# DLR-RM/curvature

Measured on AMD Instinct MI355X. Metric: KFAC factor-build + invert + sample throughput, higher is better.
Workload: dtype f32

## Files before the change

### curvature_amd/csrc/invert.hip

```cpp
#include <type_traits>
#include "kernarg.h"
#include "mma64.h"
#include <hip/hip_ext.h>

#include <algorithm>
#include <chrono>
#include <cstdlib>
#include <mutex>
#include <vector>

namespace curv {

constexpr int INV_THREADS = MMA_THREADS;
constexpr int SQ_FLAGS = 32;
constexpr int SQ_FD = 0, SQ_FLC = 4, SQ_FLROW = 8, SQ_FT = 12;
constexpr int SQ_SPIN_LIMIT = 1 << 21;
#ifdef CURV_SQ_TRACE
__device__ long long g_sq_trace[256];
#define KT_BEGIN(slot) { if (threadIdx.x == 0 && k0 == 4 * (CURV_SQ_TRACE - 1)) atomicMax((unsigned long long*)&g_sq_trace[slot], (1ull << 62) - (unsigned long long)wall_clock64()); }
#define KT_END(slot) { if (threadIdx.x == 0 && k0 == 4 * (CURV_SQ_TRACE - 1)) atomicMax((unsigned long long*)&g_sq_trace[slot], (unsigned long long)wall_clock64()); }
#define SQT(slot) { if (threadIdx.x == 0 && f == 0 && stamp == CURV_SQ_TRACE) g_sq_trace[slot] = wall_clock64(); }
#define FIT(k) { if (threadIdx.x == 0 && trace_base >= 0) g_sq_trace[trace_base + (k)] = wall_clock64(); }
#else
#define SQT(slot)
// ... 786 lines not shown
__device__ __forceinline__ void sq_wait(int* flag, int stamp, int* lost) {
  if (threadIdx.x == 0) {
    int n = 0;
    while (__hip_atomic_load(flag, __ATOMIC_RELAXED, __HIP_MEMORY_SCOPE_AGENT) < stamp) {
      __builtin_amdgcn_s_sleep(2);
      if (++n > SQ_SPIN_LIMIT || *lost) { *lost = 1; break; }
    }
  }
  __syncthreads();
}

__global__ void __launch_bounds__(INV_THREADS)
chol_square_kernel(const InvDev* __restrict__ t, int nf, int k0, int kend, int* __restrict__ flags, int stamp) {
  __shared__ double Ds[NB * LDA], Is[NB * LDA], Bf[NB * LDA];
  __shared__ int bad, lost;
  int f, r;
  if (!locate(t, nf, blockIdx.x, [k0, kend](const InvDev& d) { return d.P > k0 ? (kend < d.P ? kend : d.P) - k0 : 0; }, f, r))
    return;
  const InvDev& d = t[f];
  const int np = d.np, tid = threadIdx.x;
  const int nbf = (kend < d.P ? kend : d.P) - k0;
  gdouble* W = (gdouble*)d.W;
  gdouble* X = (gdouble*)d.X;
  int* fl = flags + (long long)f * SQ_FLAGS;
  const int lane = tid & 63, wave = tid >> 6, wm = wave >> 1, wn = wave & 1;
  auto Wt = [&](int i, int j) { return W + (long long)(k0 + i) * NB * np + (k0 + j) * NB; };
  auto Xt = [&](int i, int j) { return X + (long long)(k0 + i) * NB * np + (k0 + j) * NB; };
  if (tid == 0) { bad = 0; lost = 0; }
  __syncthreads();
  f64x4 acc[2][2];
  if (r == 0) {
    SQT(0)
#ifdef CURV_SQ_TRACE
    if (tid == 0 && f == 0 && stamp == CURV_SQ_TRACE + 1) g_sq_trace[238] = wall_clock64();
#endif
    load_block(Wt(0, 0), np, Ds);
    if (nbf > 1) load_block(Wt(1, 0), np, Bf);
    __syncthreads();
    SQT(1)
    for (int q = 0; q < nbf; ++q) {
      if (q >= 1) {
        if (q >= 2) {
          sq_wait(fl + SQ_FT + q, stamp, &lost);
          SQT(8 * q + 0)
          load_block_coh(Wt(q, q - 1), np, Bf);
        }
        load_block_coh(Wt(q, q), np, Ds);
        __syncthreads();
        SQT(8 * q + 1)
        zero_acc(acc);
        mma_64_pre<true>(Bf, Is, wm, wn, lane, acc);
        SQT(8 * q + 2)
        store_acc_coh(Wt(q, q - 1), np, acc, wm, wn, lane, 1.0);
        __syncthreads();
        acc_to_lds(acc, wm, wn, lane, Bf);
        __syncthreads();
        zero_acc(acc);
        mma_64_pre<true>(Bf, Bf, wm, wn, lane, acc);
        lds_sub_acc(Ds, acc, wm, wn, lane);
        SQT(8 * q + 3)
        sq_signal(fl + SQ_FLC + q, stamp);
        SQT(8 * q + 4)
      }
#ifdef CURV_SQ_TRACE
      factor_invert_64(Ds, Is, &bad, (k0 + q) * NB, d.pivot_min, (f == 0 && stamp == CURV_SQ_TRACE) ? 112 + 4 * q : -1);
#else
      factor_invert_64(Ds, Is, &bad, (k0 + q) * NB, d.pivot_min);
#endif
      SQT(q == 0 ? 2 : 8 * q + 5)
      store_block_coh(Xt(q, q), np, Is);
      sq_signal(fl + SQ_FD + q, stamp);
      SQT(q == 0 ? 3 : 8 * q + 6)
    }
    if (tid == 0 && bad != 0) atomicCAS(d.info, 0, bad);
    if (tid == 0 && lost != 0) atomicCAS(d.info, 0, -1);
    return;
  }
  double* Af = Ds;
  SQT(64 * r + 0)
  double* Cf = Is;
  if (r >= 2) {
    f64x4 accA[2][2], accT0[2][2], accT1[2][2];
    zero_acc(accA); zero_acc(accT0); zero_acc(accT1);
    auto push = [&](int mp, int m) {
      load_block_coh(Wt(mp, m), np, Bf);
      __syncthreads();
      if (mp == 1) mma_64_pre<true>(Cf, Bf, wm, wn, lane, accT0);
      else mma_64_pre<true>(Cf, Bf, wm, wn, lane, accT1);
      __syncthreads();
    };
    for (int m = 0; m <= r - 2; ++m) {
      SQT(64 * r + 8 + 4 * m)
      load_block(Wt(r, m), np, Af);
      __syncthreads();
      if (m == 1) lds_sub_acc(Af, accT0, wm, wn, lane);
      sq_wait(fl + SQ_FD + m, stamp, &lost);
      SQT(64 * r + 9 + 4 * m)
      load_block_coh(Xt(m, m), np, Bf);
      __syncthreads();
      zero_acc(acc);
      mma_64_pre<true>(Af, Bf, wm, wn, lane, acc);
      SQT(64 * r + 10 + 4 * m)
      store_acc_coh(Wt(r, m), np, acc, wm, wn, lane, 1.0);
      acc_to_lds(acc, wm, wn, lane, Cf);
      if (m == r - 2) sq_signal(fl + SQ_FLROW + r, stamp);
      else __syncthreads();
      mma_64_pre<true>(Cf, Cf, wm, wn, lane, accA);
      __syncthreads();
      for (int mp = m + 1; mp <= r - 1; ++mp) {
        if (m == r - 2 && mp == r - 1) break;
        sq_wait(fl + (mp == m + 1 ? SQ_FLC : SQ_FLROW) + mp, stamp, &lost);
        push(mp, m);
      }
    }
    load_block(Wt(r, r), np, Bf);
    __syncthreads();
    lds_sub_acc(Bf, accA, wm, wn, lane);
    __syncthreads();
    store_block_coh(Wt(r, r), np, Bf);
    load_block(Wt(r, r - 1), np, Af);
    sq_wait(fl + SQ_FLC + r - 1, stamp, &lost);
    push(r - 1, r - 2);
    if (r == 2) lds_sub_acc(Af, accT0, wm, wn, lane);
    else lds_sub_acc(Af, accT1, wm, wn, lane);
    __syncthreads();
    store_block_coh(Wt(r, r - 1), np, Af);
    sq_signal(fl + SQ_FT + r, stamp);
    SQT(64 * r + 1)
  }
  {
    const int j = r - 1;
    for (int i = r; i < nbf; ++i) {
      f64x4 S[2][2];
      zero_acc(S);
      for (int m = j; m < i; ++m) {
        if (m == i - 1) sq_wait(fl + SQ_FLC + i, stamp, &lost);
        else sq_wait(fl + SQ_FLROW + i, stamp, &lost);
        if (m == j) sq_wait(fl + SQ_FD + j, stamp, &lost);
        load_block_coh(Wt(i, m), np, Af);
        load_block_coh(Xt(m, j), np, Bf);
        __syncthreads();
        mma_64_pre<false>(Af, Bf, wm, wn, lane, S);
        __syncthreads();
      }
      SQT(64 * r + 2 + 16 * (i - r))
      acc_to_lds(S, wm, wn, lane, Af);
      sq_wait(fl + SQ_FD + i, stamp, &lost);
      SQT(64 * r + 3 + 16 * (i - r))
      load_block_coh(Xt(i, i), np, Bf);
      __syncthreads();
      zero_acc(acc);
      mma_64_pre<false>(Bf, Af, wm, wn, lane, acc);
      store_acc_coh(Xt(i, j), np, acc, wm, wn, lane, -1.0);
      asm volatile("s_waitcnt vmcnt(0)" ::: "memory");
      __syncthreads();
      SQT(64 * r + 4 + 16 * (i - r))
    }
  }
  if (tid == 0 && lost != 0) atomicCAS(d.info, 0, -1);
}

__device__ __host__ __forceinline__ int panel_jobs(int P, int kind, int k0, int kend) {
  if (P <= k0) return 0;
  return (P > kend ? P - kend : 0) + (kind == 2 ? (kend < P ? kend : P) : kind == 1 ? k0 : 0);
}
template <int WV>
__device__ __forceinline__ void panel_product_body(const InvDev* __restrict__ t, int nf, int k0, int kend,
                                                   double* __restrict__ As, double* __restrict__ Bs) {
  int f, local;
  if (!locate(t, nf, blockIdx.x, [k0, kend](const InvDev& d) { return panel_jobs(d.P, s_kind(d), k0, kend); }, f, local))
    return;
  const InvDev& d = t[f];
  const int np = d.np, nb = (kend < d.P ? kend : d.P) - k0;
  gdouble* W = (gdouble*)d.W;
  gdouble* X = (gdouble*)d.X;
  TileJob o;
  o.np = np;
  o.same = false;
  o.ke0 = 0;
  const int n_below = d.P > kend ? d.P - kend : 0;
  const bool below = local < n_below;
  const int i = kend + local, j = local - n_below;
  o.bt = below;
  o.mode = below ? 1 : 3;
  gdouble* Zm = (gdouble*)d.Zm;
  const bool rhs = !below && Zm != nullptr;
  gdouble* S = rhs ? Zm : X;
  if (rhs) { o.mode = 1; o.ke0 = (j > k0 ? j - k0 : 0) * NB; }
  gfloat* C32 = below ? (gfloat*)d.C32 : nullptr;
  for (int c = nb - 1; c >= 0; --c) {
    if (rhs && k0 + c < j) break;
    const gdouble* xsq = X + (long long)(k0 + c) * NB * np + k0 * NB;
    o.a0 = below ? (const gbyte*)(W + (long long)i * NB * np + k0 * NB) : (const gbyte*)xsq;
    o.b0 = below ? (const gbyte*)xsq : (const gbyte*)(S + (long long)k0 * NB * np + j * NB);
    o.C = below ? W + (long long)i * NB * np + (k0 + c) * NB : S + (long long)(k0 + c) * NB * np + j * NB;
    o.C32 = C32 != nullptr ? C32 + (long long)i * NB * np + (k0 + c) * NB : nullptr;
    o.ke1 = (c + 1) * NB;
    tile_product_k32<WV>(o, As, Bs);
  }
}

constexpr int PQ_PITCH = 4 * NB + 1;
constexpr int PQ_OWN = 16 * PQ_PITCH > 4 * NB * 17 ? 16 * PQ_PITCH : 4 * NB * 17;
template <bool below>
__device__ __forceinline__ void panel_quarter_body(const InvDev& d, int k0, int nb, int i, int j, int q,
                                                   double* __restrict__ Own, double* __restrict__ Ts) {
  const int np = d.np;
  const int tid = threadIdx.x, lane = tid & 63, wave = tid >> 6, r16 = lane & 15, kq = lane >> 4;
  PQT(240)
  const gbyte* Wb = (const gbyte*)d.W;
  const gbyte* Xb = (const gbyte*)d.X;
  if (below) {
    const gbyte* g = Wb + (((long long)i * NB + 16 * q) * np + (long long)k0 * NB) * 8;
    for (int v = 0; v < nb; ++v) {
      double x[4];
#pragma unroll
      for (int u = 0; u < 4; ++u) x[u] = *(const gdouble*)(g + ((long long)((tid >> 6) + 4 * u) * np + (tid & 63) + 64 * v) * 8);
#pragma unroll
      for (int u = 0; u < 4; ++u) Own[((tid >> 6) + 4 * u) * PQ_PITCH + (tid & 63) + 64 * v] = x[u];
    }
  } else {
    const gbyte* g = Xb + ((long long)k0 * NB * np + (long long)j * NB + 16 * q) * 8;
    for (int v = 0; v < nb; ++v) {
      double x[4];
#pragma unroll
      for (int u = 0; u < 4; ++u) {
        x[u] = *(const gdouble*)(g + ((long long)((tid >> 4) + 16 * u + 64 * v) * np + (tid & 15)) * 8);
      }
#pragma unroll
      for (int u = 0; u < 4; ++u) Own[((tid >> 4) + 16 * u + 64 * v) * 17 + (tid & 15)] = x[u];
    }
  }
  double rt0[16], rt1[16], rt2[16];
  auto fetch = [&](int c, int kb, double (&rt)[16]) __attribute__((always_inline)) {
    const gbyte* g = Xb + (((long long)(k0 + c) * NB) * np + (long long)(k0 + kb) * NB) * 8;
#pragma unroll
    for (int u = 0; u < 16; ++u) rt[u] = *(const gdouble*)(g + ((long long)((tid >> 6) + 4 * u) * np + (tid & 63)) * 8);
  };
  auto next = [](int& c, int& kb) { if (++kb > c) { --c; kb = 0; } };
  int c = nb - 1, kb = 0;
  int cf = c, kf = kb;
  fetch(cf, kf, rt0); next(cf, kf);
  if (cf >= 0) { fetch(cf, kf, rt1); next(cf, kf); }
  if (cf >= 0) { fetch(cf, kf, rt2); next(cf, kf); }
  f64x4 acc[4] = {};
  PQT(241)
  [[maybe_unused]] int pq_n = 0;
  auto step = [&](double (&rt)[16]) __attribute__((always_inline)) {
    __syncthreads();
#pragma unroll
    for (int u = 0; u < 16; ++u) Ts[((tid >> 6) + 4 * u) * LDA + (tid & 63)] = rt[u];
    __syncthreads();
    if (cf >= 0) { fetch(cf, kf, rt); next(cf, kf); }
#pragma unroll
    for (int ks = 0; ks < NB / 4; ++ks) {
      const int k = 4 * ks + kq;
      const double a = below ? Own[r16 * PQ_PITCH + 64 * kb + k] : Ts[(16 * wave + r16) * LDA + k];
      const double b = below ? Ts[(16 * wave + r16) * LDA + k] : Own[(64 * kb + k) * 17 + r16];
      acc[ks & 3] = __builtin_amdgcn_mfma_f64_16x16x4f64(a, b, acc[ks & 3], 0, 0, 0);
    }
    if (kb == c) {
      const int wm = below ? q : wave, wn = below ? wave : q;
      const int c16 = lane & 15, rq = lane >> 4;
      gbyte* base = below ? (gbyte*)d.W + (((long long)i * NB) * np + (long long)(k0 + c) * NB) * 8
                          : (gbyte*)d.X + (((long long)(k0 + c) * NB) * np + (long long)j * NB) * 8;
      const unsigned voff = (unsigned)(((long long)(16 * wm + rq) * np + 16 * wn + c16) * 8);
      gbyte* base32 = (below && d.C32 != nullptr) ? (gbyte*)d.C32 + (((long long)i * NB) * np + (long long)(k0 + c) * NB) * 4 : nullptr;
      const unsigned voff32 = (unsigned)(((long long)(16 * wm + rq) * np + 16 * wn + c16) * 4);
#pragma unroll
      for (int qq = 0; qq < 4; ++qq) {
        const double v = (acc[0][qq] + acc[1][qq]) + (acc[2][qq] + acc[3][qq]);
        *(gdouble*)(base + (long long)(4 * qq) * np * 8 + voff) = below ? v : -v;
        if (below && base32 != nullptr) *(gfloat*)(base32 + (long long)(4 * qq) * np * 4 + voff32) = (float)v;
      }
#pragma unroll
      for (int u = 0; u < 4; ++u) acc[u] = f64x4{0.0, 0.0, 0.0, 0.0};
    }
    next(c, kb);
    PQT(242 + pq_n)
    ++pq_n;
  };
  while (c >= 0) {
    step(rt0);
    if (c < 0) break;
    step(rt1);
    if (c < 0) break;
    step(rt2);
  }
}
__global__ void __launch_bounds__(INV_THREADS)
panel_product_quarter_kernel(const InvDev* __restrict__ t, int nf, int k0, int kend) {
  __shared__ double Own[PQ_OWN], Ts[NB * LDA];
  const int job = (blockIdx.x >> 5) * 8 + (blockIdx.x & 7), q = (blockIdx.x >> 3) & 3;
  int f, local;
  KT_BEGIN(236)
  if (!locate(t, nf, job, [k0, kend](const InvDev& d) { return panel_jobs(d.P, s_kind(d), k0, kend); }, f, local)) return;
  const InvDev& d = t[f];
  const int nb = (kend < d.P ? kend : d.P) - k0;
  const int n_below = d.P > kend ? d.P - kend : 0;
  if (local < n_below) panel_quarter_body<true>(d, k0, nb, kend + local, 0, q, Own, Ts);
  else panel_quarter_body<false>(d, k0, nb, 0, local - n_below, q, Own, Ts);
  KT_END(237)
}
__global__ void __launch_bounds__(INV_THREADS, 3)
panel_product_kernel(const InvDev* __restrict__ t, int nf, int k0, int kend) {
  __shared__ double As[NB * OPA], Bs[NB * OPA > OKS * LDA ? NB * OPA : OKS * LDA];
  panel_product_body<2>(t, nf, k0, kend, As, Bs);
}
__global__ void __launch_bounds__(1024)
panel_product_wide_kernel(const InvDev* __restrict__ t, int nf, int k0, int kend) {
  __shared__ double As[NB * OPA], Bs[NB * OPA > OKS * LDA ? NB * OPA : OKS * LDA];
  panel_product_body<4>(t, nf, k0, kend, As, Bs);
}

constexpr int SKS = 32;
constexpr int SPA = SKS + 1;
constexpr int SPB = NB + 32;
struct Tile32 {
  const gbyte* a;
  const gbyte* b;
  gfloat* out;
  int np, ke0, ke1;
  bool a64, b64, accumulate, negate;
};
__device__ __forceinline__ void tile32(const Tile32& o, float* __restrict__ As, float* __restrict__ Bs) {
  const int np = o.np;
  const int tid = threadIdx.x, lane = tid & 63, wave = tid >> 6, wm = wave >> 1, wn = wave & 1;
  const int l32 = lane & 31, h = lane >> 5;
  const long long a_off = (long long)(tid >> 3) * np + 4 * (tid & 7), a_step = 32ll * np;
  const long long b_off = (long long)(tid >> 4) * np + 4 * (tid & 15), b_step = 16ll * np;
  typedef const __attribute__((address_space(1))) f32x4 gf4;
  typedef const __attribute__((address_space(1))) f64x4 gd4;
  f32x4 ra[2], rb[2];
  auto fetch = [&](int ke) __attribute__((always_inline)) {
    if (o.a64) {
#pragma unroll
      for (int u = 0; u < 2; ++u) {
        const f64x4 v = *(gd4*)(o.a + (a_off + u * a_step + ke) * 8);
        ra[u] = f32x4{(float)v[0], (float)v[1], (float)v[2], (float)v[3]};
      }
    } else {
#pragma unroll
      for (int u = 0; u < 2; ++u) ra[u] = *(gf4*)(o.a + (a_off + u * a_step + ke) * 4);
    }
    if (o.b64) {
#pragma unroll
      for (int u = 0; u < 2; ++u) {
        const f64x4 v = *(gd4*)(o.b + (b_off + u * b_step + (long long)ke * np) * 8);
        rb[u] = f32x4{(float)v[0], (float)v[1], (float)v[2], (float)v[3]};
      }
    } else {
#pragma unroll
      for (int u = 0; u < 2; ++u) rb[u] = *(gf4*)(o.b + (b_off + u * b_step + (long long)ke * np) * 4);
    }
  };
  f32x16 acc = {0};
  fetch(o.ke0);
  for (int ke = o.ke0; ke < o.ke1; ke += SKS) {
#pragma unroll
    for (int u = 0; u < 2; ++u)
#pragma unroll
      for (int e = 0; e < 4; ++e) {
        As[((tid >> 3) + 32 * u) * SPA + 4 * (tid & 7) + e] = ra[u][e];
        Bs[((tid >> 4) + 16 * u) * SPB + 4 * (tid & 15) + e] = rb[u][e];
      }
    __syncthreads();
    if (ke + SKS < o.ke1) fetch(ke + SKS);
#pragma unroll
    for (int kk = 0; kk < SKS; kk += 2) {
      const float av = As[(32 * wm + l32) * SPA + kk + h];
      const float bv = Bs[(kk + h) * SPB + 32 * wn + l32];
      acc = __builtin_amdgcn_mfma_f32_32x32x2f32(av, bv, acc, 0, 0, 0);
    }
    __syncthreads();
  }
  gbyte* base = (gbyte*)(o.out + (long long)(32 * wm + 4 * h) * np + 32 * wn + l32);
  if (!o.accumulate) {
#pragma unroll
    for (int reg = 0; reg < 16; ++reg)
      *(gfloat*)(base + (long long)((reg & 3) + 8 * (reg >> 2)) * np * 4) = o.negate ? -acc[reg] : acc[reg];
  } else {
    float old[16];
#pragma unroll
    for (int reg = 0; reg < 16; ++reg) old[reg] = *(const gfloat*)(base + (long long)((reg & 3) + 8 * (reg >> 2)) * np * 4);
#pragma unroll
    for (int reg = 0; reg < 16; ++reg) *(gfloat*)(base + (long long)((reg & 3) + 8 * (reg >> 2)) * np * 4) = old[reg] + acc[reg];
  }
}
__device__ __host__ __forceinline__ long long supd_tiles(int P, int kind, int kend) {
  if (kind != 0 || P <= kend) return 0;
  const long long nsb = (P - kend + SB - 1) / SB, ncb = (kend + SB - 1) / SB;
  return nsb * ncb * (SB * SB);
}
__global__ void __launch_bounds__(INV_THREADS, 3)
supd32_kernel(const InvDev* __restrict__ t, int nf, int k0, int kend, int n_items) {
  __shared__ float As[NB * SPA], Bs[SKS * SPB];
  int item;
  {
    const int bid = blockIdx.x, xcd = bid & 7, jj = bid >> 3;
    item = ((jj / (SB * SB)) * 8 + xcd) * (SB * SB) + (jj % (SB * SB));
  }
  if (item >= n_items) return;
  int f, local;
  if (!locate(t, nf, item, [kend](const InvDev& d) { return (int)supd_tiles(d.P, s_kind(d), kend); }, f, local)) return;
  const InvDev& d = t[f];
  const int np = d.np, r = d.P - kend;
  const int ncb = (kend + SB - 1) / SB;
  const int sb = local / (SB * SB), in = local - sb * (SB * SB);
  const int a = sb / ncb, cb = sb - a * ncb;
  const int ri = a * SB + in / SB, j = cb * SB + in % SB;
  if (ri >= r || j >= kend) return;
  const int i = kend + ri;
  const bool own = j >= k0;
  Tile32 o;
  o.np = np;
  o.a = (const gbyte*)((const gfloat*)d.C32 + (long long)i * NB * np);
  o.a64 = false;
  o.b = own ? (const gbyte*)((const gdouble*)d.X + j * NB) : (const gbyte*)((const gfloat*)d.X32 + j * NB);
  o.b64 = own;
  o.ke0 = (own ? j : k0) * NB;
  o.ke1 = kend * NB;
  o.out = (gfloat*)d.S32 + (long long)i * NB * np + j * NB;
  o.accumulate = !own;
  o.negate = false;
  tile32(o, As, Bs);
}
__device__ __host__ __forceinline__ long long xrow_tiles(int P, int kind, int k0, int kend) {
  if (kind != 0 || P <= k0) return 0;
  return (long long)((kend < P ? kend : P) - k0) * k0;
}
__global__ void __launch_bounds__(INV_THREADS, 3)
xrows32_kernel(const InvDev* __restrict__ t, int nf, int k0, int kend) {
  __shared__ float As[NB * SPA], Bs[SKS * SPB];
  int f, local;
  if (!locate(t, nf, blockIdx.x, [k0, kend](const InvDev& d) { return (int)xrow_tiles(d.P, s_kind(d), k0, kend); }, f, local)) return;
  const InvDev& d = t[f];
  const int np = d.np, nb = (kend < d.P ? kend : d.P) - k0;
  const int j = local / nb, c = nb - 1 - (local - j * nb);
  Tile32 o;
  o.np = np;
  o.a = (const gbyte*)((const gdouble*)d.X + (long long)(k0 + c) * NB * np);
  o.a64 = true;
  o.b = (const gbyte*)((const gfloat*)d.S32 + j * NB);
  o.b64 = false;
  o.ke0 = k0 * NB;
  o.ke1 = (k0 + c + 1) * NB;
  o.out = (gfloat*)d.X32 + (long long)(k0 + c) * NB * np + j * NB;
  o.accumulate = false;
  o.negate = true;
  tile32(o, As, Bs);
}

__global__ void __launch_bounds__(INV_THREADS)
inv_finalize_kernel(const InvDev* __restrict__ t, int nf, int sq) {
  __shared__ float tile[NB][NB + 1];
  int f, local;
  if (!locate(t, nf, blockIdx.x, [](const InvDev& d) { return d.P * d.P; }, f, local)) return;
  const InvDev& d = t[f];
  const int n = d.n, np = d.np, q = d.P;
  const int ti = local / q, tj = local - ti * q;
  const gdouble* X = (const gdouble*)d.X;
  const gfloat* X32 = (const gfloat*)d.X32;
  gfloat* L = (gfloat*)d.L;
  const int w = __builtin_amdgcn_readfirstlane(threadIdx.x >> 6), c = threadIdx.x & 63;
  if (!d.reverse) {
    gdouble* Xo = (gdouble*)d.Xout;
    const gdouble* S = d.Zm != nullptr ? (const gdouble*)d.Zm : X;
#pragma unroll 4
    for (int u = 0; u < 16; ++u) {
      const int i = ti * NB + w + 4 * u, j = tj * NB + c;
      if (i < n && j < n) {
        double v = (j <= i) ? S[(long long)i * np + j] : 0.0;
        if (d.r_minus && j <= i) v = ((const gdouble*)d.R)[(long long)i * n + j] - v;
        Xo[(long long)i * n + j] = v;
      }
    }
    return;
  }
  if (tj > ti) {
#pragma unroll 4
    for (int u = 0; u < 16; ++u) {
      const int i = ti * NB + w + 4 * u, j = tj * NB + c;
      if (i < n && j < n) L[(long long)i * n + j] = 0.0f;
    }
    return;
  }
  double xv[16];
  const int i_l = ti * NB + c;
#pragma unroll
  for (int u = 0; u < 16; ++u) {
    const int j = tj * NB + w + 4 * u;
    const int rs = n - 1 - j, cs = n - 1 - i_l;
    const bool live = i_l < n && j < n && j <= i_l;
    if (X32 == nullptr || rs / sq == cs / sq) xv[u] = live ? X[(long long)rs * np + cs] : 0.0;
    else xv[u] = live ? (double)X32[(long long)rs * np + cs] : 0.0;
  }
#pragma unroll
  for (int u = 0; u < 16; ++u) tile[w + 4 * u][c] = (float)xv[u];
  __syncthreads();
#pragma unroll
  for (int u = 0; u < 16; ++u) {
    const int i = ti * NB + w + 4 * u, j = tj * NB + c;
    if (i < n && j < n) L[(long long)i * n + j] = tile[c][w + 4 * u];
  }
}

constexpr int INV_UPLOAD_CHUNK = 28;

static size_t inv_table_bytes(int n) { return align_up((size_t)std::max(n, 1) * sizeof(InvDev), 256); }
static size_t inv_flags_bytes(int n) { return align_up((size_t)std::max(n, 1) * SQ_FLAGS * sizeof(int), 256); }

struct SideStream {
  hipStream_t stream = nullptr;
  hipEvent_t ev_main[2] = {nullptr, nullptr};
  hipEvent_t ev_side[2] = {nullptr, nullptr};
  hipEvent_t ev_tail = nullptr;
};
struct StreamSet {
  SideStream side[2];
  hipStream_t aux = nullptr;
  hipStream_t masked = nullptr;
  hipEvent_t ev_fork = nullptr, ev_join = nullptr, ev_join2 = nullptr;
  hipEvent_t ev_chain[2] = {nullptr, nullptr};
};
static std::mutex g_masked_mutex;
static std::vector<std::pair<int, hipStream_t>> g_masked_streams;
static void destroy_masked_streams() {
  std::lock_guard<std::mutex> lock(g_masked_mutex);
  for (auto& e : g_masked_streams) {
    if (hipSetDevice(e.first) == hipSuccess) {
      (void)hipStreamSynchronize(e.second);
      (void)hipStreamDestroy(e.second);
    }
  }
  g_masked_streams.clear();
}

static int stream_set(StreamSet** out) {
  static thread_local std::vector<std::pair<int, StreamSet>> cache;
  int dev = 0;
  CURV_HIP_CHECK(hipGetDevice(&dev));
  for (auto& e : cache) if (e.first == dev) { *out = &e.second; return CURV_OK; }
  StreamSet s;
  int prio_low = 0, prio_high = 0;
  CURV_HIP_CHECK(hipDeviceGetStreamPriorityRange(&prio_low, &prio_high));
  CURV_HIP_CHECK(hipEventCreateWithFlags(&s.ev_fork, hipEventDisableTiming));
  CURV_HIP_CHECK(hipEventCreateWithFlags(&s.ev_join, hipEventDisableTiming));
  CURV_HIP_CHECK(hipEventCreateWithFlags(&s.ev_join2, hipEventDisableTiming));
  for (int g = 0; g < 2; ++g) CURV_HIP_CHECK(hipEventCreateWithFlags(&s.ev_chain[g], hipEventDisableTiming));
  auto wide_stream = [&](hipStream_t* out) -> int {
    static const int free_cus = getenv("CURV_FREE_CUS") ? atoi(getenv("CURV_FREE_CUS")) : 32;
    hipDeviceProp_t prop;
    int dev_id = 0;
    CURV_HIP_CHECK(hipGetDevice(&dev_id));
    CURV_HIP_CHECK(hipGetDeviceProperties(&prop, dev_id));
    const int n_cu = prop.multiProcessorCount;
    if (free_cus > 0 && 2 * free_cus <= n_cu) {
      std::vector<uint32_t> mask((size_t)cdiv(n_cu, 32), 0u);
      for (int c = 0; c < n_cu - free_cus; ++c) mask[c >> 5] |= 1u << (c & 31);
      if (hipExtStreamCreateWithCUMask(out, (uint32_t)mask.size(), mask.data()) == hipSuccess) {
        std::lock_guard<std::mutex> lock(g_masked_mutex);
        if (g_masked_streams.empty()) atexit(destroy_masked_streams);
        g_masked_streams.emplace_back(dev_id, *out);
        return CURV_OK;
      }
      (void)hipGetLastError();
    }
    CURV_HIP_CHECK(hipStreamCreateWithPriority(out, hipStreamNonBlocking, prio_low));
    return CURV_OK;
  };
  CURV_HIP_CHECK(hipStreamCreateWithPriority(&s.aux, hipStreamNonBlocking, prio_high));
  CURV_HIP_CHECK(hipStreamCreateWithFlags(&s.masked, hipStreamNonBlocking));
  for (int g = 0; g < 2; ++g) {
    { const int rc = wide_stream(&s.side[g].stream); if (rc != CURV_OK) return rc; }
    for (int i = 0; i < 2; ++i) {
      CURV_HIP_CHECK(hipEventCreateWithFlags(&s.side[g].ev_main[i], hipEventDisableTiming));
      CURV_HIP_CHECK(hipEventCreateWithFlags(&s.side[g].ev_side[i], hipEventDisableTiming));
    }
    CURV_HIP_CHECK(hipEventCreateWithFlags(&s.side[g].ev_tail, hipEventDisableTiming));
  }
  cache.emplace_back(dev, s);
  *out = &cache.back().second;
  return CURV_OK;
}

int curv_internal_side_stream(hipStream_t* out) {
  StreamSet* ss = nullptr;
  const int rc = stream_set(&ss);
  if (rc != CURV_OK) return rc;
  *out = ss->masked;
  return CURV_OK;
}

}

using namespace curv;

#ifdef CURV_SQ_TRACE
extern "C" int curv_debug_sq_trace_reset() {
  long long zeros[256] = {0};
  return hipMemcpyToSymbol(HIP_SYMBOL(curv::g_sq_trace), zeros, sizeof(zeros)) == hipSuccess ? 0 : 1;
}
extern "C" int curv_debug_sq_trace(long long* out) {
  return hipMemcpyFromSymbol(out, HIP_SYMBOL(curv::g_sq_trace), 256 * sizeof(long long)) == hipSuccess ? 0 : 1;
}
#endif

extern "C" int curv_init_streams(void) {
  StreamSet* ss = nullptr;
  return stream_set(&ss);
}

extern "C" size_t curv_chol_inv_workspace_bytes(const curv_inv_desc* descs, int n_factors) {
  size_t total = 2 * inv_table_bytes(n_factors) + 2 * inv_flags_bytes(n_factors);
  for (int i = 0; i < n_factors; ++i) {
    if (descs[i].n <= 0) return 0;
    const size_t np = (size_t)cdiv(descs[i].n, NB) * NB;
    total += 2 * np * np * sizeof(double) + 3 * np * np * sizeof(float);
  }
  return total;
}

static int sweep_nbo(bool latency_bound) { return latency_bound ? 4 : 6; }
struct GroupSweep {
  hipStream_t stream;
  SideStream* side;
  const std::vector<InvDev>* tabp;
  InvDev* table;
  int* flags;
  bool latency_bound;
  int n_factors = 0, Pmax = 0, NBO = 4, k0 = 0, panel = 0;
  long long fin_tiles = 0, quarter_prod = 0;
  bool use_square = false, far_pending = false, inv_pending = false, capturing = false;

  GroupSweep(hipStream_t st, SideStream* sd, const std::vector<InvDev>& tab, InvDev* tb, int* fl, bool lb)
      : stream(st), side(sd), tabp(&tab), table(tb), flags(fl), latency_bound(lb) {}
  bool done() const { return k0 >= Pmax; }
  int panels() const { return cdiv(Pmax, NBO); }

  int begin() {
    const std::vector<InvDev>& tab = *tabp;
    n_factors = (int)tab.size();
    hipStreamCaptureStatus cap = hipStreamCaptureStatusNone;
    CURV_HIP_CHECK(hipStreamIsCapturing(stream, &cap));
    capturing = cap != hipStreamCaptureStatusNone;
    long long prep_tiles = 0;
    for (const InvDev& d : tab) {
      Pmax = std::max(Pmax, d.P);
      prep_tiles += (long long)d.P * (d.P + 1) / 2;
      fin_tiles += (long long)d.P * d.P;
    }
    const int rcu = upload_table<INV_UPLOAD_CHUNK>(stream, table, tab.data(), n_factors);
    if (rcu != CURV_OK) return rcu;
    hipLaunchKernelGGL(inv_prepare_kernel, dim3((unsigned)prep_tiles), dim3(INV_THREADS), 0, stream, table, n_factors, flags);
    CURV_LAUNCH_CHECK();
    NBO = sweep_nbo(latency_bound);
    return CURV_OK;
  }

  int panel_step() {
    const std::vector<InvDev>& tab = *tabp;
    constexpr long long WIDE_NEAR = 512, WIDE_PROD = 256;
    constexpr long long QUARTER_PROD = 512;
    quarter_prod = latency_bound ? QUARTER_PROD : 0;
    use_square = latency_bound;
    const int kend = k0 + NBO, row0 = kend + NBO;
    long long prod_tiles = 0;
    if (use_square) {
      long long sq_wgs = 0;
      for (const InvDev& d : tab)
        if (d.P > k0) sq_wgs += std::min(kend, d.P) - k0;
      hipLaunchKernelGGL(chol_square_kernel, dim3((unsigned)sq_wgs), dim3(INV_THREADS), 0, stream, table, n_factors, k0, kend,
                         flags, panel + 1);
      CURV_LAUNCH_CHECK();
    }
    for (int k = k0; !use_square && k < std::min(kend, Pmax); ++k) {
      long long diag_tiles = 0, panel_tiles = 0, upd_tiles = 0;
      for (const InvDev& d : tab) {
        if (d.P > k) { ++diag_tiles; panel_tiles += std::min(kend, d.P) - k0 - 1; }
        upd_tiles += inner_tiles(d.P, k, k0, kend);
      }
      if (k == k0) {
        hipLaunchKernelGGL(chol_diag_kernel, dim3((unsigned)diag_tiles), dim3(INV_THREADS), 0, stream, table, n_factors, k);
        CURV_LAUNCH_CHECK();
      }
      if (panel_tiles > 0) {
        hipLaunchKernelGGL(chol_panel_kernel, dim3((unsigned)panel_tiles), dim3(INV_THREADS), 0, stream, table, n_factors, k, k0, kend);
        CURV_LAUNCH_CHECK();
      }
      if (upd_tiles > 0) {
        hipLaunchKernelGGL(inner_update_kernel, dim3((unsigned)upd_tiles), dim3(INV_THREADS), 0, stream, table, n_factors, k, k0, kend);
        CURV_LAUNCH_CHECK();
      }
    }
    auto launch_product = [&](hipStream_t st, long long jobs, hipEvent_t done) -> int {
      const InvDev* tb = table;
      if (jobs <= quarter_prod)
        hipExtLaunchKernelGGL(panel_product_quarter_kernel, dim3((unsigned)(cdivll(jobs, 8) * 32)), dim3(INV_THREADS), 0, st,
                              nullptr, done, 0, tb, n_factors, k0, kend);
      else if (jobs <= WIDE_PROD)
        hipExtLaunchKernelGGL(panel_product_wide_kernel, dim3((unsigned)jobs), dim3(1024), 0, st, nullptr, done, 0, tb, n_factors,
                              k0, kend);
      else
        hipExtLaunchKernelGGL(panel_product_kernel, dim3((unsigned)jobs), dim3(INV_THREADS), 0, st, nullptr, done, 0, tb,
                              n_factors, k0, kend);
      CURV_LAUNCH_CHECK();
      return CURV_OK;
    };
    long long inv_jobs = 0, inv_tiles = 0;
    for (const InvDev& d : tab) {
      prod_tiles += panel_jobs(d.P, s_kind(d), k0, kend);
      inv_jobs += xrow_tiles(d.P, s_kind(d), k0, kend);
      inv_tiles += supd_tiles(d.P, s_kind(d), kend);
    }
    bool fork_recorded = false;
    if (prod_tiles > 0) {
      fork_recorded = !capturing;
      const int rc = launch_product(stream, prod_tiles, fork_recorded ? side->ev_main[panel & 1] : nullptr);
      if (rc != CURV_OK) return rc;
    }
    long long near_tiles = 0, far_tiles = 0;
    for (const InvDev& d : tab) {
      near_tiles += strip_tiles(d.P, kend, kend, row0, s_in_sweep(d));
      far_tiles += outer_tiles(d.P, kend, row0, s_in_sweep(d));
    }
    hipStream_t inv_st = side->stream;
    const bool inv_work = inv_jobs > 0 || inv_tiles > 0;
    const bool side_work = far_tiles > 0 || inv_work;
    if (side_work) {
      if (!fork_recorded) CURV_HIP_CHECK(hipEventRecord(side->ev_main[panel & 1], stream));
      CURV_HIP_CHECK(hipStreamWaitEvent(side->stream, side->ev_main[panel & 1], 0));
    }
    if (near_tiles > 0) {
      if (far_pending) {
        CURV_HIP_CHECK(hipStreamWaitEvent(stream, side->ev_side[(panel + 1) & 1], 0));
      }
      far_pending = false;
      if (near_tiles <= WIDE_NEAR)
        hipLaunchKernelGGL(outer_update_wide_kernel, dim3((unsigned)near_tiles), dim3(1024), 0, stream, table, n_factors,
                           k0, kend, kend, row0, 1, (int)near_tiles);
      else
        hipLaunchKernelGGL(outer_update_kernel, dim3((unsigned)near_tiles), dim3(INV_THREADS), 0, stream, table, n_factors, k0,
                           kend, kend, row0, 1, (int)near_tiles);
      CURV_LAUNCH_CHECK();
    }
    if (far_tiles > 0) {
      const bool ride = !capturing;
      const InvDev* tb = table;
      long long trail = 0;
      for (const InvDev& d : tab) trail += outer_tiles(d.P, kend, row0, false);
      const long long s_tiles = far_tiles - trail;
      if (trail > 0) {
        const long long g1 = cdivll(trail, 8 * SB * SB) * 8 * SB * SB;
        hipExtLaunchKernelGGL(outer_update_dma_kernel, dim3((unsigned)g1), dim3(INV_THREADS), 0, side->stream, nullptr,
                              (ride && s_tiles == 0) ? side->ev_side[panel & 1] : nullptr, 0, tb, n_factors, k0, kend, row0, (int)trail);
        CURV_LAUNCH_CHECK();
      }
      if (s_tiles > 0) {
        const long long g2 = cdivll(s_tiles, 8 * SB * SB) * 8 * SB * SB;
        hipExtLaunchKernelGGL(outer_update_kernel, dim3((unsigned)g2), dim3(INV_THREADS), 0, side->stream, nullptr,
                              ride ? side->ev_side[panel & 1] : nullptr, 0, tb, n_factors, k0, kend, row0, 0, 2, (int)s_tiles);
        CURV_LAUNCH_CHECK();
      }
      if (!ride) CURV_HIP_CHECK(hipEventRecord(side->ev_side[panel & 1], side->stream));
      far_pending = true;
    }
    if (inv_jobs > 0) {
      hipLaunchKernelGGL(xrows32_kernel, dim3((unsigned)inv_jobs), dim3(INV_THREADS), 0, inv_st, table, n_factors, k0, kend);
      CURV_LAUNCH_CHECK();
      inv_pending = true;
    }
    if (inv_tiles > 0) {
      const long long grid = cdivll(inv_tiles, 8 * SB * SB) * 8 * SB * SB;
      hipLaunchKernelGGL(supd32_kernel, dim3((unsigned)grid), dim3(INV_THREADS), 0, inv_st, table, n_factors, k0, kend,
                         (int)inv_tiles);
      CURV_LAUNCH_CHECK();
      inv_pending = true;
    }
    k0 += NBO;
    ++panel;
    return CURV_OK;
  }

  int end(hipEvent_t chain_done = nullptr) {
    if (chain_done != nullptr) CURV_HIP_CHECK(hipEventRecord(chain_done, stream));
    if (far_pending) CURV_HIP_CHECK(hipStreamWaitEvent(stream, side->ev_side[(panel + 1) & 1], 0));
    if (inv_pending) {
      CURV_HIP_CHECK(hipEventRecord(side->ev_tail, side->stream));
      CURV_HIP_CHECK(hipStreamWaitEvent(stream, side->ev_tail, 0));
    }
    hipLaunchKernelGGL(inv_finalize_kernel, dim3((unsigned)fin_tiles), dim3(INV_THREADS), 0, stream, table, n_factors, NBO * NB);
    CURV_LAUNCH_CHECK();
    return CURV_OK;
  }
};

static int chol_sweep_group(hipStream_t stream, SideStream* side, const std::vector<InvDev>& tab, InvDev* table, int* flags,
                            bool latency_bound, hipEvent_t chain_done = nullptr) {
  GroupSweep g(stream, side, tab, table, flags, latency_bound);
  int rc = g.begin();
  while (rc == CURV_OK && !g.done()) rc = g.panel_step();
  return rc == CURV_OK ? g.end(chain_done) : rc;
}

constexpr int SPLIT_P = 16;

struct EarlyStatus { int* host; const int* dev; size_t bytes; hipEvent_t ev; };

static int await_verdict(const EarlyStatus* early) {
  if (early != nullptr) CURV_HIP_CHECK(hipEventSynchronize(early->ev));
  return CURV_OK;
}

static int chol_sweep(hipStream_t stream, std::vector<InvDev>& tab, void* workspace, size_t workspace_bytes,
                      const char* who, const EarlyStatus* early = nullptr) {
  const int n_factors = (int)tab.size();
  static const int latency_max = getenv("CURV_LATENCY_MAX") ? atoi(getenv("CURV_LATENCY_MAX")) : 64;
  bool any_rhs = false;
  for (const InvDev& d : tab) any_rhs = any_rhs || d.R != nullptr;
  const bool latency_bound = n_factors <= latency_max && !any_rhs;
  size_t need = 2 * inv_table_bytes(n_factors) + 2 * inv_flags_bytes(n_factors);
  for (const InvDev& d : tab)
    need += (d.R != nullptr ? 3 : 2) * (size_t)d.np * d.np * sizeof(double) + (d.reverse ? 3 * (size_t)d.np * d.np * sizeof(float) : 0);
  if (workspace == nullptr || workspace_bytes < need) {
    set_error("%s: workspace too small (%zu < %zu bytes)", who, workspace_bytes, need);
    return CURV_ERR_WORKSPACE;
  }
  char* p = reinterpret_cast<char*>(workspace) + 2 * inv_table_bytes(n_factors);
  int* flags0 = reinterpret_cast<int*>(p);
  int* flags1 = reinterpret_cast<int*>(p + inv_flags_bytes(n_factors));
  p += 2 * inv_flags_bytes(n_factors);
  std::vector<InvDev> big, small;
  int Pmax = 0;
  for (const InvDev& d : tab) Pmax = std::max(Pmax, d.P);
  const int split = std::max(SPLIT_P, Pmax / 2);
  for (InvDev& d : tab) {
    d.W = reinterpret_cast<double*>(p); p += (size_t)d.np * d.np * sizeof(double);
    d.X = reinterpret_cast<double*>(p); p += (size_t)d.np * d.np * sizeof(double);
    if (d.R != nullptr) { d.Zm = reinterpret_cast<double*>(p); p += (size_t)d.np * d.np * sizeof(double); }
    if (d.reverse) {
      d.C32 = reinterpret_cast<float*>(p); p += (size_t)d.np * d.np * sizeof(float);
      d.X32 = reinterpret_cast<float*>(p); p += (size_t)d.np * d.np * sizeof(float);
      d.S32 = reinterpret_cast<float*>(p); p += (size_t)d.np * d.np * sizeof(float);
    }
    (d.P > split || latency_bound ? big : small).push_back(d);
  }
  StreamSet* ss = nullptr;
  { const int rc = stream_set(&ss); if (rc != CURV_OK) return rc; }
  InvDev* table0 = reinterpret_cast<InvDev*>(workspace);
  InvDev* table1 = reinterpret_cast<InvDev*>(reinterpret_cast<char*>(workspace) + inv_table_bytes(n_factors));
  hipStreamCaptureStatus capture = hipStreamCaptureStatusNone;
  CURV_HIP_CHECK(hipStreamIsCapturing(stream, &capture));
  if (capture != hipStreamCaptureStatusNone) {
    if (early != nullptr) {
      set_error("%s: the early status read-back is a host copy and cannot be captured", who);
      return CURV_ERR_INVALID;
    }
    if (!big.empty()) {
      const int rc = chol_sweep_group(stream, &ss->side[0], big, table0, flags0, latency_bound);
      if (rc != CURV_OK) return rc;
    }
    if (!small.empty()) return chol_sweep_group(stream, &ss->side[1], small, big.empty() ? table0 : table1,
                                                big.empty() ? flags0 : flags1, latency_bound);
    return CURV_OK;
  }
  if (big.empty() || small.empty()) {
    CURV_HIP_CHECK(hipEventRecord(ss->ev_fork, stream));
    CURV_HIP_CHECK(hipStreamWaitEvent(ss->aux, ss->ev_fork, 0));
    const int rc1 = chol_sweep_group(ss->aux, &ss->side[0], big.empty() ? small : big, table0, flags0, latency_bound,
                                     early ? ss->ev_chain[0] : nullptr);
    if (rc1 != CURV_OK) return rc1;
    if (early != nullptr) {
      CURV_HIP_CHECK(hipStreamWaitEvent(ss->side[0].stream, ss->ev_chain[0], 0));
      CURV_HIP_CHECK(hipMemcpyAsync(early->host, early->dev, early->bytes, hipMemcpyDeviceToHost, ss->side[0].stream));
      CURV_HIP_CHECK(hipEventRecord(early->ev, ss->side[0].stream));
    }
    { const int rc = await_verdict(early); if (rc != CURV_OK) return rc; }
    CURV_HIP_CHECK(hipEventRecord(ss->ev_join, ss->aux));
    CURV_HIP_CHECK(hipStreamWaitEvent(stream, ss->ev_join, 0));
    return CURV_OK;
  }
  CURV_HIP_CHECK(hipEventRecord(ss->ev_fork, stream));
  CURV_HIP_CHECK(hipStreamWaitEvent(ss->aux, ss->ev_fork, 0));
  CURV_HIP_CHECK(hipStreamWaitEvent(ss->masked, ss->ev_fork, 0));
  constexpr int START_FRAC = 30;
  const int n_panels = cdiv(Pmax, sweep_nbo(latency_bound));
  long long far0 = 0;
  for (const InvDev& d : big) far0 += outer_tiles(d.P, 4, 8, s_in_sweep(d));
  const int start_panel = far0 >= 5000 ? std::min(n_panels - 1, n_panels * START_FRAC / 100) : 0;
  GroupSweep gb(ss->aux, &ss->side[0], big, table0, flags0, latency_bound);
  GroupSweep gs(ss->masked, &ss->side[1], small, table1, flags1, latency_bound);
  int rc = gb.begin();
  if (rc != CURV_OK) return rc;
  bool small_started = false;
  for (int t = 0; !gb.done() || !small_started || !gs.done(); ++t) {
    if (!small_started && (t >= start_panel || gb.done())) {
      if (t > 0) {
        CURV_HIP_CHECK(hipEventRecord(ss->ev_join2, ss->aux));
        CURV_HIP_CHECK(hipStreamWaitEvent(ss->masked, ss->ev_join2, 0));
      }
      rc = gs.begin();
      if (rc != CURV_OK) return rc;
      small_started = true;
    }
    if (!gb.done()) { rc = gb.panel_step(); if (rc != CURV_OK) return rc; }
    if (small_started && !gs.done()) { rc = gs.panel_step(); if (rc != CURV_OK) return rc; }
  }
  rc = gb.end(early ? ss->ev_chain[0] : nullptr);
  if (rc != CURV_OK) return rc;
  rc = gs.end(early ? ss->ev_chain[1] : nullptr);
  if (rc != CURV_OK) return rc;
  if (early != nullptr) {
    CURV_HIP_CHECK(hipStreamWaitEvent(ss->side[1].stream, ss->ev_chain[0], 0));
    CURV_HIP_CHECK(hipStreamWaitEvent(ss->side[1].stream, ss->ev_chain[1], 0));
    CURV_HIP_CHECK(hipMemcpyAsync(early->host, early->dev, early->bytes, hipMemcpyDeviceToHost, ss->side[1].stream));
    CURV_HIP_CHECK(hipEventRecord(early->ev, ss->side[1].stream));
  }
  { const int rc = await_verdict(early); if (rc != CURV_OK) return rc; }
  CURV_HIP_CHECK(hipEventRecord(ss->ev_join, ss->aux));
  CURV_HIP_CHECK(hipStreamWaitEvent(stream, ss->ev_join, 0));
  CURV_HIP_CHECK(hipEventRecord(ss->ev_join2, ss->masked));
  CURV_HIP_CHECK(hipStreamWaitEvent(stream, ss->ev_join2, 0));
  return CURV_OK;
}

static int chol_inv_lower_impl(void* stream_, const curv_inv_desc* descs, int n_factors, int* info,
                               void* workspace, size_t workspace_bytes, const EarlyStatus* early);

constexpr int INV_MAX_N = 1 << 21;

extern "C" int curv_chol_inv_lower(void* stream_, const curv_inv_desc* descs, int n_factors, int* info,
                                   void* workspace, size_t workspace_bytes) {
  return chol_inv_lower_impl(stream_, descs, n_factors, info, workspace, workspace_bytes, nullptr);
}

extern "C" int curv_chol_inv_lower_status(void* stream_, const curv_inv_desc* descs, int n_factors, int* info,
                                          void* workspace, size_t workspace_bytes, int* host_status, void* ev_status) {
  CURV_REQUIRE(host_status != nullptr && ev_status != nullptr, "curv_chol_inv_lower_status: null argument");
  if (n_factors == 0) return CURV_OK;
  EarlyStatus early{host_status, info, (size_t)n_factors * sizeof(int), (hipEvent_t)ev_status};
  return chol_inv_lower_impl(stream_, descs, n_factors, info, workspace, workspace_bytes, &early);
}

static int chol_inv_lower_impl(void* stream_, const curv_inv_desc* descs, int n_factors, int* info,
                               void* workspace, size_t workspace_bytes, const EarlyStatus* early) {
  if (n_factors == 0) return CURV_OK;
  CURV_REQUIRE(descs != nullptr && info != nullptr, "curv_chol_inv_lower: null argument");
  std::vector<InvDev> tab(n_factors);
  for (int i = 0; i < n_factors; ++i) {
    const curv_inv_desc& s = descs[i];
    CURV_REQUIRE(s.n > 0, "curv_chol_inv_lower: factor %d: empty", i);
    CURV_REQUIRE(s.n <= INV_MAX_N, "curv_chol_inv_lower: factor %d: %d wide, the sweep takes at most %d", i, s.n, INV_MAX_N);
    CURV_REQUIRE(s.F != nullptr && s.L != nullptr, "curv_chol_inv_lower: factor %d: null pointer", i);
    CURV_REQUIRE(s.multiply >= 0.0 && s.add >= 0.0, "curv_chol_inv_lower: factor %d: negative hyper-parameter", i);
    InvDev& d = tab[i];
    memset(&d, 0, sizeof(d));
    d.F = s.F; d.L = s.L; d.n = s.n;
    d.P = cdiv(s.n, NB); d.np = d.P * NB;
    d.info = info + i;
    d.sqrt_s = (float)sqrt(s.multiply);
    d.sqrt_n = (float)sqrt(s.add);
    d.reverse = 1;
  }
  return chol_sweep((hipStream_t)stream_, tab, workspace, workspace_bytes, "curv_chol_inv_lower", early);
}

extern "C" size_t curv_chol_factor_inverse_workspace_bytes(const curv_cholinv_desc* descs, int n) {
  size_t total = 2 * inv_table_bytes(n) + 2 * inv_flags_bytes(n);
  for (int i = 0; i < n; ++i) {
    if (descs[i].n <= 0) return 0;
    const size_t np = (size_t)cdiv(descs[i].n, NB) * NB;
    total += (descs[i].R != nullptr ? 3 : 2) * np * np * sizeof(double);
  }
  return total;
}

extern "C" int curv_chol_factor_inverse(void* stream_, const curv_cholinv_desc* descs, int n_mats, int* info,
                                        void* workspace, size_t workspace_bytes) {
  if (n_mats == 0) return CURV_OK;
  CURV_REQUIRE(descs != nullptr && info != nullptr, "curv_chol_factor_inverse: null argument");
  std::vector<InvDev> tab(n_mats);
  for (int i = 0; i < n_mats; ++i) {
    const curv_cholinv_desc& s = descs[i];
    CURV_REQUIRE(s.n <= INV_MAX_N, "curv_chol_factor_inverse: matrix %d: %d wide, the sweep takes at most %d", i, s.n,
                 INV_MAX_N);
    CURV_REQUIRE(s.n > 0 && s.M != nullptr && s.X != nullptr, "curv_chol_factor_inverse: matrix %d invalid", i);
    InvDev& d = tab[i];
    memset(&d, 0, sizeof(d));
    d.F = reinterpret_cast<const float*>(s.M); d.Xout = s.X; d.n = s.n;
    d.f64_in = s.m_is_f64 ? 1 : 0;
    d.P = cdiv(s.n, NB); d.np = d.P * NB;
    d.info = info + i;
    d.sqrt_s = 1.0f;
    d.sqrt_n = (float)s.diag_add;
    d.reverse = 0;
    d.pivot_min = s.pivot_min > 0.0 ? s.pivot_min : 0.0;
    d.R = s.R;
    d.r_minus = (s.R != nullptr && s.r_minus) ? 1 : 0;
  }
  return chol_sweep((hipStream_t)stream_, tab, workspace, workspace_bytes, "curv_chol_factor_inverse");
// ... 2 lines not shown
```

Before: 4129.

## Add row-split panel product kernel for small KFAC-only panel sweeps

Adds a specialised panel product kernel for NBO=6 that splits each row job across four workgroups. Each workgroup stages its slice of the W row in shared memory and streams X triangle tiles through a three-deep register prefetch ring feeding f64 MFMA. It writes both the f64 and f32 outputs directly. The kernel is selected only when the sweep is not latency bound, all factors are plain KFAC, and the job count is small, aiming to raise parallelism and cut launch or occupancy overhead for small panels. The cost is more code paths and a quadrant-based tiling that must match the existing layout.

```diff
diff --git a/curvature_amd/csrc/invert.hip b/curvature_amd/csrc/invert.hip
--- a/curvature_amd/csrc/invert.hip
+++ b/curvature_amd/csrc/invert.hip
@@ -1112,6 +1112,73 @@
   else panel_quarter_body<false>(d, k0, nb, 0, local - n_below, q, Own, Ts);
   KT_END(237)
 }
+constexpr int PR_NB = 6;
+typedef double f64x2 __attribute__((ext_vector_type(2)));
+typedef const __attribute__((address_space(1))) f64x2 gd2;
+constexpr int pr_tile_c(int nbw, int T) { int c = nbw - 1; while (T > c) { T -= c + 1; --c; } return c; }
+constexpr int pr_tile_kb(int nbw, int T) { int c = nbw - 1; while (T > c) { T -= c + 1; --c; } return T; }
+template <int NBW>
+__global__ void __launch_bounds__(INV_THREADS, 3)
+panel_product_rows_kernel(const InvDev* __restrict__ t, int nf, int k0) {
+  __shared__ f64x2 Own[NBW * (NB / 2) * 16];
+  constexpr int NT = NBW * (NBW + 1) / 2;
+  const int kend = k0 + NBW;
+  const int job = (blockIdx.x >> 5) * 8 + (blockIdx.x & 7), q = (blockIdx.x >> 3) & 3;
+  int f, local;
+  if (!locate(t, nf, job, [k0, kend](const InvDev& d) { return panel_jobs(d.P, 0, k0, kend); }, f, local)) return;
+  const InvDev& d = t[f];
+  const int np = d.np, i = kend + local;
+  const int tid = threadIdx.x, lane = tid & 63, wave = tid >> 6, r16 = lane & 15, kq = lane >> 4;
+  {
+    const gbyte* g = (const gbyte*)d.W + (((long long)i * NB + 16 * q + (tid & 15)) * np + (long long)k0 * NB + 2 * (tid >> 4)) * 8;
+#pragma unroll
+    for (int v = 0; v < 2 * NBW; v += 2) {
+      f64x2 x[2];
+#pragma unroll
+      for (int u = 0; u < 2; ++u) x[u] = *(gd2*)(g + (v + u) * 256);
+#pragma unroll
+      for (int u = 0; u < 2; ++u) Own[((tid >> 4) + 16 * (v + u)) * 16 + (tid & 15)] = x[u];
+    }
+  }
+  f64x2 rt[3][8];
+  const gbyte* xsq = (const gbyte*)d.X + (((long long)k0 * NB + 16 * wave + r16) * np + (long long)k0 * NB + 2 * kq) * 8;
+  auto fetch = [&](int c, int kb, f64x2 (&r)[8]) __attribute__((always_inline)) {
+    const gbyte* g = xsq + ((long long)c * NB * np + kb * NB) * 8;
+#pragma unroll
+    for (int u = 0; u < 8; ++u) r[u] = *(gd2*)(g + u * 64);
+  };
+#pragma unroll
+  for (int T = 0; T < 3 && T < NT; ++T) fetch(pr_tile_c(NBW, T), pr_tile_kb(NBW, T), rt[T]);
+  f64x4 acc[4] = {};
+  __syncthreads();
+  const long long el = ((long long)i * NB + 16 * q + (lane >> 4)) * np + (long long)k0 * NB + 16 * wave + (lane & 15);
+  gbyte* out = (gbyte*)d.W + el * 8;
+  gbyte* out32 = (gbyte*)d.C32 + el * 4;
+#pragma unroll
+  for (int T = 0; T < NT; ++T) {
+    const int c = pr_tile_c(NBW, T), kb = pr_tile_kb(NBW, T);
+    const f64x2* own = Own + (32 * kb + kq) * 16 + r16;
+#pragma unroll
+    for (int u = 0; u < 8; ++u) {
+      const f64x2 a = own[u * 64];
+      acc[(2 * u) & 3] = __builtin_amdgcn_mfma_f64_16x16x4f64(a.x, rt[T % 3][u].x, acc[(2 * u) & 3], 0, 0, 0);
+      acc[(2 * u + 1) & 3] = __builtin_amdgcn_mfma_f64_16x16x4f64(a.y, rt[T % 3][u].y, acc[(2 * u + 1) & 3], 0, 0, 0);
+    }
+    __builtin_amdgcn_sched_barrier(0);
+    if (T + 3 < NT) fetch(pr_tile_c(NBW, T + 3), pr_tile_kb(NBW, T + 3), rt[T % 3]);
+    __builtin_amdgcn_sched_barrier(0);
+    if (kb == c) {
+#pragma unroll
+      for (int qq = 0; qq < 4; ++qq) {
+        const double v = (acc[0][qq] + acc[1][qq]) + (acc[2][qq] + acc[3][qq]);
+        *(gdouble*)(out + ((long long)(4 * qq) * np + c * NB) * 8) = v;
+        *(gfloat*)(out32 + ((long long)(4 * qq) * np + c * NB) * 4) = (float)v;
+      }
+#pragma unroll
+      for (int u = 0; u < 4; ++u) acc[u] = f64x4{0.0, 0.0, 0.0, 0.0};
+    }
+  }
+}
 __global__ void __launch_bounds__(INV_THREADS, 3)
 panel_product_kernel(const InvDev* __restrict__ t, int nf, int k0, int kend) {
   __shared__ double As[NB * OPA], Bs[NB * OPA > OKS * LDA ? NB * OPA : OKS * LDA];
@@ -1440,8 +1507,8 @@
   int* flags;
   bool latency_bound;
   int n_factors = 0, Pmax = 0, NBO = 4, k0 = 0, panel = 0;
-  long long fin_tiles = 0, quarter_prod = 0;
-  bool use_square = false, far_pending = false, inv_pending = false, capturing = false;
+  long long fin_tiles = 0, quarter_prod = 0, rows_prod = 0;
+  bool use_square = false, far_pending = false, inv_pending = false, capturing = false, kfac_only = true;
 
   GroupSweep(hipStream_t st, SideStream* sd, const std::vector<InvDev>& tab, InvDev* tb, int* fl, bool lb)
       : stream(st), side(sd), tabp(&tab), table(tb), flags(fl), latency_bound(lb) {}
@@ -1457,6 +1524,7 @@
     long long prep_tiles = 0;
     for (const InvDev& d : tab) {
       Pmax = std::max(Pmax, d.P);
+      kfac_only = kfac_only && s_kind(d) == 0;
       prep_tiles += (long long)d.P * (d.P + 1) / 2;
       fin_tiles += (long long)d.P * d.P;
     }
@@ -1473,6 +1541,8 @@
     constexpr long long WIDE_NEAR = 512, WIDE_PROD = 256;
     constexpr long long QUARTER_PROD = 512;
     quarter_prod = latency_bound ? QUARTER_PROD : 0;
+    constexpr long long ROWS_PROD = 192;
+    rows_prod = (!latency_bound && kfac_only && NBO == PR_NB) ? ROWS_PROD : 0;
     use_square = latency_bound;
     const int kend = k0 + NBO, row0 = kend + NBO;
     long long prod_tiles = 0;
@@ -1505,7 +1575,10 @@
     }
     auto launch_product = [&](hipStream_t st, long long jobs, hipEvent_t done) -> int {
       const InvDev* tb = table;
-      if (jobs <= quarter_prod)
+      if (jobs <= rows_prod)
+        hipExtLaunchKernelGGL(panel_product_rows_kernel<PR_NB>, dim3((unsigned)(cdivll(jobs, 8) * 32)), dim3(INV_THREADS), 0, st,
+                              nullptr, done, 0, tb, n_factors, k0);
+      else if (jobs <= quarter_prod)
         hipExtLaunchKernelGGL(panel_product_quarter_kernel, dim3((unsigned)(cdivll(jobs, 8) * 32)), dim3(INV_THREADS), 0, st,
                               nullptr, done, 0, tb, n_factors, k0, kend);
       else if (jobs <= WIDE_PROD)
```

Measured after the change: 4082. -1.1%, worse.
